# phlash/java-sdr

Hardware: AMD Instinct MI355X
Metric: IQ Msamples/s through FFT+FIR+BPSK demod, 2048-pt frames (higher is better)
Workload: dtype f64

## Files before the change

### include/jsdr_hip.h

```cpp
#ifndef JSDR_HIP_H
#define JSDR_HIP_H

#include <stddef.h>
#include <stdint.h>

#ifdef __cplusplus
extern "C" {
#endif

#define JSDR_OK 0
#define JSDR_ERR (-1)

const char *jsdr_last_error(void);
int jsdr_version(void);
int jsdr_device_count(int *count);
int jsdr_set_device(int device);
int jsdr_get_device(int *device);
int jsdr_device_name(char *buf, int cap);
int jsdr_malloc(void **dev, size_t bytes);
int jsdr_free(void *dev);
int jsdr_live_resources(int64_t *device_buffers, int64_t *device_bytes, int64_t *pinned_buffers, int64_t *streams_and_events);
int jsdr_memset(void *dev, int value, size_t bytes);
int jsdr_memcpy_h2d(void *dev, const void *host, size_t bytes);
int jsdr_memcpy_d2h(void *host, const void *dev, size_t bytes);
// ... 94 lines not shown
int jsdr_bpsk_blob_info(const void *blob_host, size_t bytes, jsdr_bpsk_blob_info_t *out);
int jsdr_bpsk_state_kernel_ms(jsdr_bpsk *h, double *pack_ms, double *unpack_ms);
int jsdr_bpsk_acq_last_launch(jsdr_bpsk *h, int64_t *fwd_frames, int64_t *inv_frames);
int jsdr_bpsk_channel_info(jsdr_bpsk *h, int *ninputs, int *nchannels);
int jsdr_bpsk_set_channel_tuning(jsdr_bpsk *h, int channel, double tuning_hz);
int jsdr_bpsk_set_channel_mode(jsdr_bpsk *h, int channel, int do_fft, int do_up);
int jsdr_bpsk_get_channel_control(jsdr_bpsk *h, int channel, double *tuning_hz, int *do_fft, int *do_up);
int jsdr_bpsk_receive_f32(jsdr_bpsk *h, const float *iq_host);
int jsdr_bpsk_receive_i16(jsdr_bpsk *h, const int16_t *raw_host, int ic, int qc);
int jsdr_bpsk_batch_i16(jsdr_bpsk *h, const int16_t *raw_dev, int64_t stream_stride_i16,
                        int64_t nsamples, int ic, int qc, void *stream);
int jsdr_bpsk_batch_f32(jsdr_bpsk *h, const float *iq_dev, int64_t stream_stride_f32, int64_t nsamples, void *stream);
int jsdr_bpsk_set_cu_share(jsdr_bpsk *h, int wgs_per_cu);
int jsdr_bpsk_pair_shares(jsdr_bpsk *h, int *fft_wgs_per_cu, int *bpsk_wgs_per_cu);
int jsdr_bpsk_last_launch(jsdr_bpsk *h, int64_t *work_items, int64_t *workgroups);
int jsdr_bpsk_sync(jsdr_bpsk *h);
enum { JSDR_BPSK_NCOUNTERS = 10 };
int jsdr_bpsk_get_counters(jsdr_bpsk *h, int stream, int32_t out[JSDR_BPSK_NCOUNTERS]);
int jsdr_bpsk_get_bits(jsdr_bpsk *h, int stream, int8_t *bits_host, int cap, int *nbits);
int jsdr_bpsk_get_fec(jsdr_bpsk *h, int stream, int idx, int32_t *rc, int32_t *bit_index, uint8_t out_host[256]);
int jsdr_bpsk_get_fec_count(jsdr_bpsk *h, int stream, int *count);
int jsdr_bpsk_get_decoded(jsdr_bpsk *h, int stream, uint8_t out_host[256]);
int jsdr_bpsk_get_trace(jsdr_bpsk *h, int stream, double *out_host, int64_t cap_pairs, int64_t *npairs);
int jsdr_bpsk_get_state(jsdr_bpsk *h, int stream, double out[18]);
typedef struct jsdr_bpsk_snapshot {
    int64_t frames;
    int32_t counters[JSDR_BPSK_NCOUNTERS];
    int32_t nbits;
    double state[18];
    uint8_t decoded[256];
// ... 92 lines not shown
```

### java-sdr_amd/binding.py

```python
import ctypes as C
import os
import re

import numpy as np

HERE = os.path.dirname(os.path.abspath(__file__))
ROOT = os.path.dirname(HERE)
_SO = os.environ.get("JSDR_LIB") or os.path.join(HERE, "libjsdr_hip.so")


class JsdrError(RuntimeError):
    pass


def library_path():
    return _SO


def _declared_symbols():
    hdr = open(os.path.join(ROOT, "include", "jsdr_hip.h")).read()
    hdr = re.sub(r"/\*.*?\*/", " ", hdr, flags=re.S)
    return sorted(set(re.findall(r"\b(jsdr_[a-z0-9_]+)\s*\(", hdr)))


# ... 361 lines not shown
def fec_decode_dev(raw_dev, nblocks, out_dev, rc_dev, stream=None):
    _check(lib().jsdr_fec_decode_batch(_addr(raw_dev), C.c_int64(nblocks), _addr(out_dev), _addr(rc_dev),
                                       C.c_void_p(stream)), "jsdr_fec_decode_batch")


COUNTER_NAMES = ["cntRaw", "cntDS", "cntBit", "cntFEC", "cntDec", "dmErrBits", "dmCorr", "dmMaxCorr", "decodeOK",
                 "centreBin"]


class BpskSnapshot(C.Structure):
    _fields_ = [("frames", C.c_int64), ("counters", C.c_int32 * 10), ("nbits", C.c_int32), ("state", C.c_double * 18),
                ("decoded", C.c_uint8 * 256), ("bits", C.c_int8 * 512)]


def bpsk_table(which):
    out = np.empty(65, np.float64)
    _check(lib().jsdr_bpsk_table(which, _addr(out), 65), "jsdr_bpsk_table")
    return out[:27 if which == 0 else 65].copy()


class Bpsk:

    def __init__(self, rate=96000, blen=8192, size=4, tuning=12000, do_fft=0, do_up=0, nstreams=1,
                 max_batch_samples=None, variant="exact"):
        self.samples = blen // size
        self.nstreams = nstreams
        self.max_batch = max_batch_samples or self.samples
        self.h = C.c_void_p()
        _check(lib().jsdr_bpsk_create(C.byref(self.h), rate, self.samples, tuning, do_fft, do_up, nstreams,
                                      C.c_int64(self.max_batch)), "jsdr_bpsk_create")
        if variant != "exact":
            _check(lib().jsdr_bpsk_set_variant(self.h, {"exact": 0, "fast": 1}[variant]), "jsdr_bpsk_set_variant")

# ... 65 lines not shown
               "jsdr_bpsk_recover_uncertified")
        return rec.value

    def set_cu_share(self, wgs_per_cu):
        _check(lib().jsdr_bpsk_set_cu_share(self.h, int(wgs_per_cu)), "jsdr_bpsk_set_cu_share")

    def pair_shares(self):
        a, b = C.c_int(), C.c_int()
        _check(lib().jsdr_bpsk_pair_shares(self.h, C.byref(a), C.byref(b)), "jsdr_bpsk_pair_shares")
        return a.value, b.value

    def last_launch(self):
        a, b = C.c_int64(), C.c_int64()
        _check(lib().jsdr_bpsk_last_launch(self.h, C.byref(a), C.byref(b)), "jsdr_bpsk_last_launch")
        return a.value, b.value

    def sync(self):
        _check(lib().jsdr_bpsk_sync(self.h), "jsdr_bpsk_sync")

    def set_tuning(self, tuning_hz):
        _check(lib().jsdr_bpsk_set_tuning(self.h, C.c_double(tuning_hz)), "jsdr_bpsk_set_tuning")

    def set_mode(self, do_fft, do_up):
        _check(lib().jsdr_bpsk_set_mode(self.h, int(do_fft), int(do_up)), "jsdr_bpsk_set_mode")

    def reconfigure(self, tuning_hz, do_fft, do_up):
        _check(lib().jsdr_bpsk_reconfigure(self.h, C.c_double(tuning_hz), int(do_fft), int(do_up)), "jsdr_bpsk_reconfigure")

    def control(self):
        t, f, u = C.c_double(), C.c_int(), C.c_int()
# ... 497 lines not shown
```

### java-sdr_amd/csrc/bpsk_fm.hip

```cpp
#include "bpsk_units.h"
#include <math.h>
#include <stddef.h>
#include <stdlib.h>

namespace jsdr {
namespace fm { __constant__ BpskConst c_bpsk; }
using fm::c_bpsk;
}
#include "bpsk_matched.h"

namespace jsdr {


template <bool FAST>
__global__ __launch_bounds__(512) void k_matched(MatchedArgs a)
{
    extern __shared__ __align__(16) unsigned char smem[];
    double2 *X = reinterpret_cast<double2 *>(smem);
    const int s = blockIdx.y;
    const long long G = a.tile0 + 4160LL * blockIdx.x;
    const double2 *dm = a.dm + (long long)s * a.dm_stride;
    {
        constexpr int NLD = (64 + 4160 + 511) / 512;
        double2 v[NLD];
// ... 115 lines not shown
    const int s = u >> 5, i = u & 31;
    if (s >= hi.nstreams || i >= 26) return;
    const long long n = hi.nsamples - 26 + i;
    int2 v;
    if (n < 0) {
        v = hi.hist_old[(long long)s * 32 + (26 + n)];
    } else {
        const int w = hi.raw[(long long)s * hi.stride_pairs + n];
        const int si = java_short_add((int)(short)(w & 0xffff), hi.ic);
        const int sq = java_short_add(w >> 16, hi.qc);
        v = make_int2((si & 0xffff) | (sq << 16), 0);
    }
    hi.hist_new[(long long)s * 32 + i] = v;
}

template <int D, int R, bool MIX, bool DC, bool FAST, bool SMALL = false>
#ifndef JSDR_FM_MINWAVES
#define JSDR_FM_MINWAVES 2
#endif
__global__ __launch_bounds__(FM_THREADS, JSDR_FM_MINWAVES) void k_fm(FmArgs a)
{
    constexpr int RD = D * R, NS = RD - D + 27, NSQ = (NS + 3) / 4;
    constexpr int JOBS = (FM_NT + R - 1) / R, ROUNDS = (JOBS + FM_THREADS - 1) / FM_THREADS;
    extern __shared__ __align__(16) unsigned char smem[];
    double2 *X = reinterpret_cast<double2 *>(smem);
    double *sc = reinterpret_cast<double *>(smem + FM_NT * sizeof(double2));
    for (int i = threadIdx.x; i < 512; i += FM_THREADS) sc[i] = a.sincos[i];
#ifdef JSDR_X_CLK
    unsigned long long clk_acc_[6] = {0, 0, 0, 0, 0, 0}, clk_last_ = 0;
#endif
    const long long nwork = (long long)a.ntiles * a.nstreams;
#pragma unroll 1
    for (long long work = blockIdx.x; work < nwork; work += gridDim.x) {
    const int s = (int)(work / a.ntiles);
    const long long G = a.tile0 + (long long)(65 * FM_NB) * (work % a.ntiles);
    const int jrel0 = (int)(G - 64 - a.g_first);
#ifdef JSDR_X_FM_SMALLSET
    const int *raw = a.raw + (long long)(s & 15) * a.stride_pairs;
// ... 4 lines not shown
    const double2 *dmh_old = a.dmh_old + (long long)s * 64;
    const int Lm1 = a.nsamples - 1, nds = a.nds, P = a.tper;
    const double HOWARD = 0.9 * 32768.0 * (double)I16_2P15_UNSCALE;
    int e0 = 0;
    if constexpr (MIX) {
        const long long v = (long long)a.first_out + (long long)D * jrel0;
        e0 = (int)(((v % P) + P) % P);
    }
    typedef const __attribute__((address_space(4))) double *const_tab_t;
    const_tab_t tb = (const_tab_t)(a.tcs + e0);
    float amx = 0.0f;
    __syncthreads();
#ifdef JSDR_X_CLK
    clk_last_ = __builtin_amdgcn_s_memtime();
#endif
#ifdef JSDR_X_NOFRONT
    if (a.nds < 0)
#endif
#pragma unroll 1
    for (int round = 0; round < ROUNDS; round++) {
        const int job = threadIdx.x + FM_THREADS * round;
        const int t0 = R * job;
        if (t0 >= FM_NT) break;
        const int j0 = jrel0 + t0;
        const int n0 = a.first_out + D * j0 - 26;
        const bool none = j0 + R <= 0 || j0 >= nds || nds <= 0;
        const bool regular = j0 >= 0 && j0 + R <= nds;
        if (!none) {
            int4 W[NSQ];
            const int *wp = raw + n0;
// ... 30 lines not shown
                if (q == 0) {
#pragma unroll
                    for (int r = 0; r < R; r++) {
                        const int kv = (kv4[r / 4] >> (8 * (r % 4))) & 0xff;
                        vc[r] = sc[kv];
                        vs[r] = sc[256 + kv];
                    }
                }
#pragma unroll
                for (int t = 3; t >= 0; t--) {
                    const int m = 4 * q + t;
                    if (m < NS) {
                        const int w = (t == 0) ? w4.x : (t == 1) ? w4.y : (t == 2) ? w4.z : w4.w;
                        double di, dq;
                        fm_convert_2p15(w, a.ic, a.qc, DC, di, dq, FAST ? &amx : nullptr);
                        if constexpr (MIX) {
                            di = di * tb[2 * m];
                            dq = dq * tb[2 * m + 1];
                        }
#pragma unroll
                        for (int r = 0; r < R; r++) {
                            if (m >= D * r && m <= D * r + 26) {
                                const int age = D * r + 26 - m;
                                const double tp = ds_tap(age);
                                const bool same = age == 0 || ((kDsPow2Mask >> age) & 1);
                                if (FAST || same) {
                                    ai[r] = __builtin_fma(di, tp, ai[r]);
                                    aq[r] = __builtin_fma(dq, tp, aq[r]);
                                } else {
                                    ai[r] += di * tp;
                                    aq[r] += dq * tp;
                                }
                            }
                        }
                    }
                }
#ifndef JSDR_FM_NOPIN
#pragma unroll
                for (int r = 0; r < R; r++) asm volatile("" : "+v"(ai[r]), "+v"(aq[r])::"memory");
                if constexpr (FAST) asm volatile("" : "+v"(amx));
                __builtin_amdgcn_sched_barrier(0);
#endif
            }
            if (regular) {
#pragma unroll
// ... 17 lines not shown
                        val.y = r == 0 ? oq[0] : r == 1 ? oq[1] : r == 2 ? oq[2] : r == 3 ? oq[3] : oq[R - 1];
                    } else if (j >= -64 && j < 0) {
                        val = dmh_old[64 + j];
                    }
                    if (t < FM_NT) X[t] = val;
                }
            }
        } else {
#pragma unroll 1
            for (int r = 0; r < R; r++) {
                const int t = t0 + r, j = j0 + r;
                const double2 val = (j >= -64 && j < 0) ? dmh_old[64 + j] : make_double2(0.0, 0.0);
                if (t < FM_NT) X[t] = val;
            }
        }
    }
    if constexpr (FAST) {
#pragma unroll
        for (int off = 32; off >= 1; off >>= 1) amx = fmaxf(amx, __shfl_xor(amx, off, 64));
        if ((threadIdx.x & 63) == 0 && amx > 0.0f) atomicMax(a.amax + s, __float_as_int(amx));
    }
    FM_CLK(1);
    __syncthreads();
    FM_CLK(3);
    if (jrel0 + FM_NT > nds - 64) {
        double2 *dmh_new = a.dmh_new + (long long)s * 64;
        for (int t = 64 + threadIdx.x; t < FM_NT; t += FM_THREADS) {
            const int j = jrel0 + t;
            if (j >= nds - 64 && j < nds && j >= 0) dmh_new[j - (nds - 64)] = X[t];
        }
// ... 121 lines not shown

int launch_dm_history(double2 *dm, long long dm_stride, long long nds, int nstreams, hipStream_t st)
{
    hipLaunchKernelGGL(k_dm_history, dim3((unsigned)nstreams), dim3(64), 0, st, dm, dm_stride, nds, nstreams);
    return launched();
}

int launch_fm_prep(const EdgeArgs &ea, const HistArgs &ha, const ScatterArgs &sc, hipStream_t st)
{
    hipLaunchKernelGGL(k_fm_prep, dim3((unsigned)(((long long)ea.nstreams * (4 * FM_EDGE + 32) + sc.bytes[0] + sc.bytes[1] + 255) / 256)),
                       dim3(256), 0, st, ea, ha, sc);
    return launched();
}

template <int D, int R>
static int launch_fm_t(const FmArgs &a_in, bool mix, bool dc, bool fast, int nstreams, hipStream_t st, long long *items, long long *grid_out)
{
    const size_t lds = (size_t)FM_NT * sizeof(double2) + 512 * sizeof(double);
    const long long span = 65LL * FM_NB;
    const long long ntiles = (a_in.g_first + a_in.nds - a_in.tile0 + span - 1) / span;
    FmArgs a = a_in;
    a.ntiles = (int)ntiles;
    a.nstreams = nstreams;
    static const long long grid_cap = [] {
        const char *e = knob("JSDR_FM_GRID");
        return e ? atoll(e) : 0LL;
    }();
    long long gx = ntiles * nstreams;
    if (grid_cap > 0 && gx > grid_cap) gx = grid_cap;
    if (a.grid_limit > 0 && gx > a.grid_limit) gx = a.grid_limit;
    *items = ntiles * nstreams;
    *grid_out = gx;
    const dim3 grid((unsigned)gx), block(FM_THREADS);
#define JSDR_FM_LAUNCH(MIX, DC, FAST, SMALL)                                                                    \
    do {                                                                                                        \
        JSDR_LDS_ATTR((k_fm<D, R, MIX, DC, FAST, SMALL>), lds);                                                 \
        hipLaunchKernelGGL((k_fm<D, R, MIX, DC, FAST, SMALL>), grid, block, lds, st, a);                        \
    } while (0)
    if (!fast && a.nds <= FM_THREADS && ntiles == 1) {
        if (mix) { if (dc) JSDR_FM_LAUNCH(true, true, false, true); else JSDR_FM_LAUNCH(true, false, false, true); }
        else { if (dc) JSDR_FM_LAUNCH(false, true, false, true); else JSDR_FM_LAUNCH(false, false, false, true); }
    } else if (fast) {
        if (mix) { if (dc) JSDR_FM_LAUNCH(true, true, true, false); else JSDR_FM_LAUNCH(true, false, true, false); }
        else { if (dc) JSDR_FM_LAUNCH(false, true, true, false); else JSDR_FM_LAUNCH(false, false, true, false); }
    } else {
        if (mix) { if (dc) JSDR_FM_LAUNCH(true, true, false, false); else JSDR_FM_LAUNCH(true, false, false, false); }
        else { if (dc) JSDR_FM_LAUNCH(false, true, false, false); else JSDR_FM_LAUNCH(false, false, false, false); }
    }
#undef JSDR_FM_LAUNCH
    return launched();
}

int launch_fm(const FmArgs &a, int decim, bool mix, bool dc, bool fast, int nstreams, hipStream_t st, long long *items, long long *grid)
{
    switch (decim) {
        case 4: return launch_fm_t<4, 5>(a, mix, dc, fast, nstreams, st, items, grid);
        case 5: return launch_fm_t<5, 4>(a, mix, dc, fast, nstreams, st, items, grid);
        case 10: return launch_fm_t<10, 4>(a, mix, dc, fast, nstreams, st, items, grid);
        case 20: return launch_fm_t<20, 4>(a, mix, dc, fast, nstreams, st, items, grid);
    }
    set_error("bpsk: unsupported decimation %d", decim);
    return JSDR_ERR;
}

void bpsk_fm_clocks_report()
{
#ifdef JSDR_X_CLK
    {
        static unsigned long long cc[256][64];
        if (hipMemcpyFromSymbol(cc, HIP_SYMBOL(g_fm_clk), sizeof(cc)) == hipSuccess) {
            static const char *nm[6] = {"-", "front half", "-", "barrier front", "matched", "barrier matched"};
            for (int i = 0; i < 6; i++) {
                if (i == 0 || i == 2) continue;
                fprintf(stderr, "k_fm clk %-16s", nm[i]);
// ... 19 lines not shown
```

### java-sdr_amd/csrc/bpsk_handle.hip

```cpp
#include "bpsk_kernels.h"
#include "bpsk_fec.h"
#include "bpsk_fft.h"
#include "bpsk_chan.h"
#include "bpsk_pst.h"
#include "bpsk_sched.h"
#include "bpsk_blob.h"
#include "bpsk_state.h"
#include <math.h>
#include <cmath>
#include <atomic>
#include <memory>
#include <thread>
#include <stddef.h>
#include <stdlib.h>
#include <vector>

static const float h_ds_half[14] = {-6.103515625000e-004F, -1.220703125000e-004F, +2.380371093750e-003F,
                                    +6.164550781250e-003F, +7.324218750000e-003F, +7.629394531250e-004F,
                                    -1.464843750000e-002F, -3.112792968750e-002F, -3.225708007813e-002F,
                                    -1.617431640625e-003F, +6.463623046875e-002F, +1.502380371094e-001F,
                                    +2.231445312500e-001F, +2.518310546875e-001F};
static const float h_dm_half[33] = {
    -0.0101130691F, -0.0086975143F, -0.0038246093F, +0.0033563764F, +0.0107237026F, +0.0157790936F, +0.0164594107F,
    +0.0119213911F, +0.0030315224F, -0.0076488191F, -0.0164594107F, -0.0197184277F, -0.0150109226F, -0.0023082460F,
// ... 49 lines not shown
    bool hist_is_float = false;
    DevBuf<int> hist_bad;
    DevBuf<int> amax;
    DevBuf<SnapPack> snap_dev;
    DevBuf<int> fm_edges;
    DevBuf<float2> fm_edges_f32;
    bool f32_batch = false;
    DevBuf<double2> dm, y[2];
    int y_cur = 0;
    DevBuf<double2> dmh[2], tcs;
    int dmh_cur = 0;
    int tab_cur = 0;
    bool halo_in_dmh = false;
    bool use_fm = true;
    long long last_fm_items = 0, last_fm_grid = 0;
    int share_wgs_per_cu = 0;
    int num_cu = 0;
    int variant = 0;
    double fast_ey = 0.0;
    double margin_scale = 1.0;
    double argmax_scale = 1.0;
    const char *front_name = "k_front";
    const char *tail_name = "k_tail";
    const char *fec_name = "k_fec_bpsk";
    bool ktu_uploaded = false;
    std::thread worker;
    bool prefetch_on = true;
    long long sched_sync = 0, sched_prefetched = 0;
    Stream tail_stream;
    Event ev_matched;
// ... 962 lines not shown
    JSDR_REQUIRE(L > 0 && L <= h->max_batch, "bpsk: nsamples=%lld outside (0, max_batch_samples=%lld]", L, h->max_batch);
    JSDR_REQUIRE((stride_i16 & 1) == 0 && (h->nstreams == 1 || stride_i16 >= 2 * L),
                 "bpsk: stream stride %lld too small for %lld samples", stride_i16, L);
    JSDR_REQUIRE(!h->do_fft || (L % h->nsf) == 0, "bpsk: FFT-acquire mode needs whole frames (%lld %% %d != 0)", L, h->nsf);
    JSDR_REQUIRE(h->variant == 0 || raw_dev, "bpsk: the fast variant takes int16 input (its certification pass re-reads the raw samples)");
    JSDR_REQUIRE(h->seam != SEAM_TO_TUNE || L >= 26, "bpsk: the first tune-mode call after FFT-acquire frames needs at least 26 samples "
                 "(the input history is rebuilt from them)");
    if (rawf_dev && h->f32_batch && h->use_fm && !h->fm_edges_f32.p && (h->decim == 4 || h->decim == 5 || h->decim == 10 || h->decim == 20))
        if (h->fm_edges_f32.alloc((size_t)h->nstreams * 4 * FM_EDGE) != JSDR_OK) return JSDR_ERR;
    if (!h->do_fft && h->seam != SEAM_TO_TUNE && hist_form(h, rawf_dev != nullptr, h->nstreams, st) != JSDR_OK) return JSDR_ERR;
    const int first_out = h->decim - 1 - h->dsCnt;
    const long long g_first = h->n_ds;
    unsigned char kh0[26], mh0[26];
    memcpy(kh0, h->h_khist, 26);
    memcpy(mh0, h->h_mhist, 26);
    const long long nds = build_schedule(h, L);
    JSDR_REQUIRE(nds <= h->max_ds, "bpsk: internal: %lld decimated samples exceed capacity %lld", nds, h->max_ds);
    const int f0 = h->cur.f0;
    const long long n0 = h->cur.n0;
    if (h->n_in == 0) memset(h->h_mhist, f0, 26);
    bool split = false;
    if (!h->do_fft) {
        split = h->cur.mix < 0 || h->seam == SEAM_TO_TUNE;
        for (int i = 0; i < 26 && !split; i++) split = h->h_mhist[i] != (unsigned char)f0;
    }
    const bool std_decim = h->decim == 4 || h->decim == 5 || h->decim == 10 || h->decim == 20;
    const int fm_rd = h->decim == 4 ? 20 : h->decim * 4;
    const bool per_ok = !h->do_fft && !split && h->cur.mix == 1 && h->cur.tper > 0 && fm_rd % h->cur.tper == 0;
    const bool fm_ok = h->use_fm && std_decim && !h->do_fft && !split && nds > 0 && L <= 0x3fffffffLL &&
                       ((raw_dev && !rawf_dev) || (rawf_dev && h->f32_batch && h->variant == 0 && h->fm_edges_f32.p)) && (h->cur.mix == 0 || per_ok);
// ... 167 lines not shown
        ma.edges = h->fm_edges.p;
        ma.tcs = tcs_p;
        ma.tper = h->cur.mix ? h->cur.tper : 1;
        ma.kvco = kvco_p;
        ma.sincos = h->sincos.p;
        ma.dmh_old = h->dmh[h->dmh_cur].p;
        ma.dmh_new = h->dmh[h->dmh_cur ^ 1].p;
        ma.y = h->y[h->y_cur].p + Y_PAD;
        ma.y_stride = h->y_stride;
        ma.nds = (int)nds;
        ma.g_first = g_first;
        ma.tile0 = first_block(g_first);
        ma.first_out = first_out;
        ma.amax = h->amax.p;
        ma.grid_limit = h->share_wgs_per_cu * h->num_cu;
        if (rawf_dev) {
            EdgeF32Args ea;
            ea.rawf = fa.rawf;
            ea.stride_pairs = fa.stride_pairs;
            ea.nsamples = (int)L;
            ea.hist = fa.hist;
            ea.edges = h->fm_edges_f32.p;
            ea.nstreams = S;
            const HistArgs ha = hist_args(h, nullptr, fa.rawf, fa.stride_pairs, L, 0, 0, S);
            ProfScope psh(h, PK_PREP, st);
            if (launch_fm_prep_f32(ea, ha, st) != JSDR_OK) return JSDR_ERR;
            hist_done = true;
        } else {
            EdgeArgs ea;
            ea.raw = fa.raw;
// ... 8 lines not shown
            const HistArgs ha = hist_args(h, fa.raw, nullptr, fa.stride_pairs, L, ic, qc, S);
            ProfScope psh(h, PK_PREP, st);
            if (launch_fm_prep(ea, ha, sc, st) != JSDR_OK) return JSDR_ERR;
            hist_done = true;
        }
        ProfScope ps(h, PK_FM, st);
        if (rawf_dev) {
            FmF32Args mf;
            mf.a = ma;
            mf.rawf = fa.rawf;
            mf.edges = h->fm_edges_f32.p;
            h->front_name = "k_fm_f32";
            if (launch_fm_f32(mf, h->decim, h->cur.mix != 0, S, st, &h->last_fm_items, &h->last_fm_grid) != JSDR_OK) return JSDR_ERR;
        } else {
        h->front_name = "k_fm";
        if (launch_fm(ma, h->decim, h->cur.mix != 0, (ic != 0) || (qc != 0), h->variant != 0, S, st, &h->last_fm_items, &h->last_fm_grid) != JSDR_OK)
            return JSDR_ERR;
        }
        h->dmh_cur ^= 1;
    } else if (nds > 0) {
        ProfScope ps(h, PK_FRONT, st);
        const bool fast = false;
        const char *front = launch_front(fa, h->decim, S, fast, st);
        if (!front) return JSDR_ERR;
        h->front_name = front;
    }
    if (!h->do_fft && hist_done) h->hist_cur ^= 1;
    if (!h->do_fft && !hist_done)
        if (run_hist_in(h, hist_args(h, fa.raw, fa.rawf, fa.stride_pairs, L, ic, qc, S), st) != JSDR_OK) return JSDR_ERR;
    const int yb = h->y_cur;
    if (wait_tail(h, yb, st) != JSDR_OK) return JSDR_ERR;
// ... 119 lines not shown
                for (int i = 0; i < 4096; i++)
                    if (w[2 * i + 1] && w[2 * i] - t0 > (e1 - t0) / 10) late++;
                fprintf(stderr, "[jsdr] k_acq_fwd %d workgroups: %d started late (> 10 %% into the launch); first end %.3f ms, last end %.3f ms after the first start\n",
                        n, late, (double)(e0 - t0) / 1e5, (double)(e1 - t0) / 1e5);
            }
        }
        long long tot = 0;
        for (int k = 0; k < 8; k++) tot += c[k];
        for (int k = 0; k < 8; k++)
            fprintf(stderr, "[jsdr] k_front_fft phase %-20s %12lld ticks  %5.1f %%\n", names[k], c[k],
                    tot ? 100.0 * (double)c[k] / (double)tot : 0.0);
    }
}

extern "C" {

int jsdr_bpsk_create(jsdr_bpsk **out, int rate, int nsamples_per_frame, int tuning_hz, int do_fft, int do_up,
                     int nstreams, int64_t max_batch_samples)
{
    JSDR_REQUIRE(out, "jsdr_bpsk_create: null handle pointer");
    *out = nullptr;
    JSDR_REQUIRE(rate >= 1, "jsdr_bpsk_create: rate %d", rate);
    const int decim = rate / 9600 > 0 ? rate / 9600 : 1;
    JSDR_REQUIRE(nsamples_per_frame > 0 && nstreams > 0 && nstreams <= 65535, "jsdr_bpsk_create: bad geometry");
    if (max_batch_samples < nsamples_per_frame) max_batch_samples = nsamples_per_frame;
    FftFront front = FRONT_NONE;
    if (do_fft) {
        int force_gen = -1;
        if (const char *e = knob("JSDR_ACQG")) force_gen = atoi(e) != 0;
        front = fft_front_kind(nsamples_per_frame, decim, false, force_gen);
// ... 49 lines not shown
              h->ds_taps_dev.alloc(32) == JSDR_OK &&
              h->dmh[0].alloc(S * 64) == JSDR_OK && h->dmh[1].alloc(S * 64) == JSDR_OK && h->hist_bad.alloc(1) == JSDR_OK && h->amax.alloc(S) == JSDR_OK && h->fm_edges.alloc(S * 4 * FM_EDGE) == JSDR_OK && h->snap_dev.alloc(1) == JSDR_OK && h->tcs.alloc(2 * (256 + FM_TABLE_SLACK)) == JSDR_OK;
    if (ok && nstreams == 1) {
        const size_t need = sizeof(float) * 2 * (size_t)nsamples_per_frame + ((size_t)h->max_batch + 26) + (size_t)h->max_ds +
                            (do_fft ? sizeof(double2) * (size_t)h->max_ds : 0) + sizeof(double2) * (256 + FM_TABLE_SLACK) + 8 * 64;
        const size_t arena = (need + 63) & ~(size_t)63;
        if (arena <= ((size_t)8 << 20) && h->pin.alloc(arena + sizeof(SnapPack))) h->pin_bytes = arena;
        else (void)hipGetLastError();
    }
    if (!ok) {
        jsdr_bpsk_destroy(h);
        return JSDR_ERR;
    }
    std::vector<double> sc(512);
    for (int n = 0; n < 256; n++) {
        double arg = n * 2.0 * TUNER_PI / 256;
        sc[n] = (double)cosl((long double)arg);
        sc[256 + n] = (double)sinl((long double)arg);
    }
    BpskConst bc;
    memset(&bc, 0, sizeof(bc));
    double sync[SYNC_N];
    (void)jsdr_bpsk_table(0, bc.ds_taps, 32);
    (void)jsdr_bpsk_table(1, bc.dm_taps, 96);
    (void)jsdr_bpsk_table(2, sync, SYNC_N);
    for (int i = 0; i < SYNC_N; i++) bc.sync[i] = sync[i] > 0.0 ? 1 : -1;
    if (do_fft) {
        if (fft_mode_alloc(h, front, false) != JSDR_OK) {
            set_error("jsdr_bpsk_create: FFT-mode initialisation failed");
            jsdr_bpsk_destroy(h);
            return JSDR_ERR;
        }
        if (const char *e = knob("JSDR_ACQ3")) h->acq_mode = atoi(e) != 0 ? 1 : 0;
// ... 151 lines not shown

int jsdr_bpsk_pair_shares(jsdr_bpsk *h, int *fft_wgs_per_cu, int *bpsk_wgs_per_cu)
{
    JSDR_REQUIRE(h && fft_wgs_per_cu && bpsk_wgs_per_cu, "jsdr_bpsk_pair_shares: null argument");
    const bool pays = !h->do_fft && h->rate == 96000 && h->nsf == 2048 && h->variant == 0 && h->nstreams >= 8192;
    *fft_wgs_per_cu = pays ? 2 : 0;
    *bpsk_wgs_per_cu = pays ? 1 : 0;
    return JSDR_OK;
}

int jsdr_bpsk_last_launch(jsdr_bpsk *h, int64_t *work_items, int64_t *workgroups)
{
    JSDR_REQUIRE(h && work_items && workgroups, "jsdr_bpsk_last_launch: null argument");
    *work_items = h->last_fm_items;
    *workgroups = h->last_fm_grid;
    return JSDR_OK;
}

int jsdr_bpsk_receive_i16(jsdr_bpsk *h, const int16_t *raw_host, int ic, int qc)
{
    JSDR_REQUIRE(h && raw_host, "jsdr_bpsk_receive_i16: null argument");
    JSDR_REQUIRE(!h->pst, "jsdr_bpsk_receive_i16: a tuned handle (jsdr_bpsk_create_tuned) takes batches only; receive() is the 1-stream "
                 "form of jsdr_bpsk_create");
    JSDR_REQUIRE(h->nstreams == 1 || (h->nch > 0 && h->nin == 1),
                 "jsdr_bpsk_receive_i16: handle has %d streams; receive() is the 1-stream form (or a 1-input channel handle)",
                 h->nstreams);
    h->pin_call = true;
    h->pin_off = 0;
    int rc = JSDR_OK;
    const size_t fb = sizeof(int16_t) * 2 * (size_t)h->nsf;
// ... 317 lines not shown
    }
    set_error("jsdr_bpsk_snapshot_read: could not get a stable copy");
    return JSDR_ERR;
}

int jsdr_bpsk_profile_enable(jsdr_bpsk *h, int on)
{
    JSDR_REQUIRE(h, "jsdr_bpsk_profile_enable: null handle");
    h->prof_on = on != 0;
    return JSDR_OK;
}

int jsdr_bpsk_table(int which, double *out, int cap)
{
    JSDR_REQUIRE(out, "jsdr_bpsk_table: null argument");
    const int n = which == 0 ? 27 : ((which == 1 || which == 2) ? 65 : 0);
    JSDR_REQUIRE(n > 0 && cap >= n, "jsdr_bpsk_table: table %d needs room for %d values", which, n);
    if (which == 0) {
        for (int i = 0; i < 14; i++) out[i] = out[26 - i] = (double)h_ds_half[i];
    } else if (which == 1) {
        for (int i = 0; i < 33; i++) out[i] = out[64 - i] = (double)h_dm_half[i];
    } else {
        int sr = 0x7f;
        for (int i = 0; i < 65; i++) {
            out[i] = (sr & 64) ? 1.0 : -1.0;
            int v = sr & 0x48;
            v ^= v >> 4;
            v ^= v >> 2;
            v ^= v >> 1;
            sr = ((sr << 1) | (v & 1)) & 0xffff;
        }
    }
    return JSDR_OK;
// ... 835 lines not shown
```

### java-sdr_amd/csrc/bpsk_kernels.h

```cpp
#pragma once
#include "common.h"
#include "bpsk_fft.h"

namespace jsdr {

enum { DS_N = 27, DM_N = 65, HIST_BITS = 5200, MIN_TRIG = 8, SYNC_N = 65 };
enum { Y_PAD = 1024 };
#ifndef JSDR_FM_NB
#define JSDR_FM_NB 62
#endif
enum { FM_NB = JSDR_FM_NB, FM_NT = 64 + 65 * FM_NB, FM_THREADS = 512, FM_TABLE_SLACK = 128, FM_EDGE = 128 };

struct BpskConst {
    double ds_taps[32];
    double dm_taps[96];
    signed char sync[72];
};
int bpsk_upload_constants(const BpskConst &bc);

struct TailState {
    double dmEnergy[8];
    double dmEnergyOut;
    double lastI, lastQ;
    double energy1, energy2;
// ... 66 lines not shown
    const double2 *tcs;
    int tper;
    const unsigned char *kvco;
    const double *sincos;
    const double2 *dmh_old;
    double2 *dmh_new;
    double2 *y;
    long long y_stride;
    int nds;
    long long g_first;
    long long tile0;
    int first_out;
    int *amax;
    int ntiles, nstreams;
    int grid_limit;
};

struct EdgeArgs {
    const int *raw;
    long long stride_pairs;
    int nsamples, ic, qc, dc;
    const int2 *hist;
    int *edges;
    int nstreams;
};
struct ScatterArgs {
    const unsigned char *src[2];
    unsigned char *dst[2];
    int bytes[2];
};
// ... 52 lines not shown

bool front_reg_enabled();
const char *launch_front(const FrontArgs &fa, int decim, int nstreams, bool fast, hipStream_t st);
int launch_front_split(const FrontArgs &fa, const unsigned short *ktu9, const double *sc9, int decim, const FftFrontState *dhist,
                       int nstreams, hipStream_t st);
int launch_seam_hist(const int2 *hist, int is_float, const double *sincos, const SeamHist &sh, FftFrontState *st, FftFrontState *st2,
                     int nstreams, hipStream_t stream);
int launch_seam_q(double2 *dm, long long dm_stride, const double2 *dm2, long long dm2_stride, int J, int nstreams, hipStream_t st);
int launch_chan_seam_hist(const int2 *hist, int is_float, const double *sc9, const ChanSeamHist &sh, FftFrontState *st, double *qcol,
                          int ninputs, hipStream_t stream);
int launch_hist_in(const HistArgs &ha, hipStream_t st);
int launch_hist_convert(int2 *hist, int nstreams, int to_float, int *bad, hipStream_t st);
int launch_matched(const MatchedArgs &ma, int nstreams, hipStream_t st);
int launch_dm_history(double2 *dm, long long dm_stride, long long nds, int nstreams, hipStream_t st);
int launch_fm_prep(const EdgeArgs &ea, const HistArgs &ha, const ScatterArgs &sc, hipStream_t st);
int launch_fm(const FmArgs &a, int decim, bool mix, bool dc, bool fast, int nstreams, hipStream_t st, long long *items, long long *grid);
int launch_fm_prep_f32(const EdgeF32Args &ea, const HistArgs &ha, hipStream_t st);
int launch_fm_f32(const FmF32Args &a, int decim, bool mix, int nstreams, hipStream_t st, long long *items, long long *grid);
const char *launch_tail(const TailArgs &ta, bool cert, hipStream_t st);
bool sync_t_applies(int max_bits);
int launch_sync_t(const SyncArgs &sa, const SyncFinArgs &sf, int nstreams, hipStream_t st);
int launch_sync(const SyncArgs &sa, long long nds, int nstreams, hipStream_t st);
int launch_sync_fin(const SyncArgs &sa, const SyncFinArgs &sf, int nstreams, hipStream_t st);
int launch_reset_maxcorr(TailState *st, int nstreams, hipStream_t stream);
int launch_reset_maxcorr_chan(TailState *st, int nin, int nch, int ch, hipStream_t stream);
int launch_pack_slots(unsigned char *slots, long long slot_bytes, int slot_bits, int trig_cap, const TailState *st, const int *nbits,
                      const signed char *bitlog, long long bitlog_stride, const int *trig_count, const int *trig_bits, const int *fec_rc,
                      const unsigned char *fec_data, const int *fec_last, const int *cnt_dec, int n_in, int n_ds, int nstreams, hipStream_t stream);
void bpsk_debug_clocks_report();

}
// ... 14 lines not shown
```

### java-sdr_amd/csrc/bpsk_sched.h

```cpp
#pragma once
#include "bpsk_tuner.h"
#include <vector>

namespace jsdr {
#pragma GCC visibility push(hidden)

enum { SCHED_HIST = 26 };

long long vco_walk(double &vco, int &ds, int decim, long long L, std::vector<unsigned char> &kvco);

struct VcoSchedule {
    bool valid = false;
    double vco0 = 0.0;
    int ds0 = 0, decim = 0;
    long long L = -1;
    double vco1 = 0.0;
    int ds1 = 0;
    std::vector<unsigned char> kvco;
};
bool vco_schedule(VcoSchedule &v, double vco, int ds, int decim, long long L);

struct ScheduleKey {
    double tu0 = 0.0, inc = 0.0, vco0 = 0.0;
    int ds0 = 0, decim = 0;
// ... 1 lines not shown
    bool do_fft = false, first = false;
    unsigned char khist0[SCHED_HIST] = {0};
    bool same_call(const ScheduleKey &o) const;
    bool operator==(const ScheduleKey &o) const { return same_call(o) && first == o.first; }
};

struct Schedule {
    bool valid = false;
    ScheduleKey key;
    double tu1 = 0.0, vco1 = 0.0;
    int ds1 = 0;
    int mix = 1;
    int f0 = 1;
    long long n0 = 0;
    int tper = 0;
    long long nds = 0;
    std::vector<unsigned char> ktu;
    std::vector<unsigned char> kvco;
    std::vector<double2> tcs;
};
enum { SCHED_TABLE_SLACK = 128 };

inline void schedule_key(Schedule &sc, const ScheduleKey &key)
{
    sc.valid = false;
    sc.key = key;
}
inline bool schedule_matches(const Schedule &sc, const ScheduleKey &key) { return sc.valid && sc.key == key; }
void compute_schedule(Schedule &sc, const double *sincos);

// ... 40 lines not shown
```

### java-sdr_amd/csrc/bpsk_sched.hip

```cpp
#include "bpsk_sched.h"
#include <thread>

namespace jsdr {

struct TunerWalk {
    double tu, inc;
    unsigned char *kt;
    long long nmix = 0;
};
template <bool TUNER>
static long long walk(TunerWalk *t, double &vco_io, int &ds_io, int decim, long long L, std::vector<unsigned char> &kvco)
{
    kvco.clear();
    kvco.reserve((size_t)(L / decim + 2));
    double tu = TUNER ? t->tu : 0.0, vco = vco_io;
    const double inc = TUNER ? t->inc : 0.0;
    int cnt = ds_io;
    long long nmix = 0;
    for (long long n = 0; n < L; n++) {
        if (TUNER) {
            tuner_advance(tu, inc);
            int k = 0;
            if (tu > 0.0) {
                k = tuner_k9(tu);
// ... 54 lines not shown
        memset(t.kt, 0, (size_t)L);
        sc.nds = walk<false>(nullptr, sc.vco1, sc.ds1, key.decim, L, sc.kvco);
    } else {
        sc.nds = walk<true>(&t, sc.vco1, sc.ds1, key.decim, L, sc.kvco);
    }
    sc.mix = (t.nmix == L) ? 1 : (t.nmix == 0 ? 0 : -1);
    sc.f0 = sc.mix == 0 ? 0 : 1;
    sc.n0 = L;
    if (sc.mix < 0) {
        double tu = key.tu0;
        sc.f0 = tuner_step(tu, key.inc) != 256;
        sc.n0 = sc.f0 ? t.nmix : L - t.nmix;
    }
    sc.tu1 = t.tu;
    sc.tper = 0;
    if (!key.do_fft && sc.mix == 1) {
        const long long off = key.first ? SCHED_HIST : 0;
        const unsigned char *k = sc.ktu.data() + off;
        const long long len = L + SCHED_HIST - off;
        const long long head = len < 1024 ? len : 1024;
        for (int p = 1; p <= 256 && p < len; p++) {
            if (!period_holds(k, head, p)) continue;
            if (period_holds(k, len, p)) {
                sc.tper = p;
                sc.tcs.resize((size_t)p + SCHED_TABLE_SLACK);
                for (int e = 0; e < p + SCHED_TABLE_SLACK; e++) {
                    const int i = (int)(((e - off) % p + p) % p);
                    const int kk = k[i];
                    sc.tcs[(size_t)e] = make_double2(sincos[kk], sincos[256 + kk]);
                }
            }
            break;
        }
    }
    sc.valid = true;
}

bool ChanKey::operator==(const ChanKey &o) const
{
    return tu0 == o.tu0 && inc == o.inc && L == o.L && first == o.first && memcmp(hist0, o.hist0, sizeof(hist0)) == 0;
}

void chan_compute(ChanSchedule &c)
{
    const long long L = c.key.L;
// ... 72 lines not shown
```

### java-sdr_amd/csrc/bpsk_tuner.h

```cpp
#pragma once
#include "common.h"

namespace jsdr {

constexpr double TUNER_PI = 3.14159265358979323846;

inline double tuner_inc(double tuning, int rate) { return 2.0 * TUNER_PI * tuning / (double)rate; }

__host__ __device__ inline void tuner_advance(double &tu, double inc)
{
    const double two_pi = 2.0 * TUNER_PI;
    tu += inc;
    if (tu > two_pi) tu -= two_pi;
}

__host__ __device__ inline int tuner_k9(double tu)
{
    const double two_pi = 2.0 * TUNER_PI;
    return tu > 0.0 ? (int)(tu * (double)256 / two_pi) % 256 : 256;
}

__host__ __device__ inline int tuner_step(double &tu, double inc)
{
    tuner_advance(tu, inc);
    return tuner_k9(tu);
}

__host__ __device__ inline int vco_step(double &vco)
{
    const double two_pi = 2.0 * TUNER_PI;
    const double vinc = 2.0 * TUNER_PI * 1200.0 / (double)9600;
    vco += vinc;
    if (vco > two_pi) vco -= two_pi;
    return (int)(vco * (double)256 / two_pi) % 256;
}

}
```

Before: 243,500.

## Specialise k_fm front-end for period-8 tuner with exact 0/±1 mixing factors

When the tuner schedule has period 8 and its factors match the quarter-rate pattern (cos/sin equal to 0 or ±1 at known phases), the host detects the rotation and launches a phase-specialised k_fm variant. That variant skips the mixing multiply for unit factors and drops the FMAs against zero factors at compile time, cutting f64 arithmetic in the decimating front end. A static_assert checks the tap exactness the FMA substitution relies on. The cost is more template instantiations and a runtime branch between two phase forms per tile. It only applies for decimation 10 with a period-8 tuner.

```diff
diff --git a/include/jsdr_hip.h b/include/jsdr_hip.h
--- a/include/jsdr_hip.h
+++ b/include/jsdr_hip.h
@@ -132,6 +132,7 @@
 int jsdr_bpsk_set_cu_share(jsdr_bpsk *h, int wgs_per_cu);
 int jsdr_bpsk_pair_shares(jsdr_bpsk *h, int *fft_wgs_per_cu, int *bpsk_wgs_per_cu);
 int jsdr_bpsk_last_launch(jsdr_bpsk *h, int64_t *work_items, int64_t *workgroups);
+int jsdr_bpsk_fm_form(jsdr_bpsk *h, int *specialised, int *phase);
 int jsdr_bpsk_sync(jsdr_bpsk *h);
 enum { JSDR_BPSK_NCOUNTERS = 10 };
 int jsdr_bpsk_get_counters(jsdr_bpsk *h, int stream, int32_t out[JSDR_BPSK_NCOUNTERS]);
diff --git a/java-sdr_amd/binding.py b/java-sdr_amd/binding.py
--- a/java-sdr_amd/binding.py
+++ b/java-sdr_amd/binding.py
@@ -399,9 +399,9 @@
 
 
 def bpsk_table(which):
-    out = np.empty(65, np.float64)
-    _check(lib().jsdr_bpsk_table(which, _addr(out), 65), "jsdr_bpsk_table")
-    return out[:27 if which == 0 else 65].copy()
+    out = np.empty(256, np.float64)
+    _check(lib().jsdr_bpsk_table(which, _addr(out), 256), "jsdr_bpsk_table")
+    return out[:{0: 27, 1: 65, 2: 65}.get(which, 256)].copy()
 
 
 class Bpsk:
@@ -497,6 +497,11 @@
         a, b = C.c_int64(), C.c_int64()
         _check(lib().jsdr_bpsk_last_launch(self.h, C.byref(a), C.byref(b)), "jsdr_bpsk_last_launch")
         return a.value, b.value
+
+    def fm_form(self):
+        a, b = C.c_int(), C.c_int()
+        _check(lib().jsdr_bpsk_fm_form(self.h, C.byref(a), C.byref(b)), "jsdr_bpsk_fm_form")
+        return bool(a.value), b.value
 
     def sync(self):
         _check(lib().jsdr_bpsk_sync(self.h), "jsdr_bpsk_sync")
diff --git a/java-sdr_amd/csrc/bpsk_fm.hip b/java-sdr_amd/csrc/bpsk_fm.hip
--- a/java-sdr_amd/csrc/bpsk_fm.hip
+++ b/java-sdr_amd/csrc/bpsk_fm.hip
@@ -1,5 +1,7 @@
 #include "bpsk_units.h"
+#include "bpsk_tuner.h"
 #include <math.h>
+#include <type_traits>
 #include <stddef.h>
 #include <stdlib.h>
 
@@ -153,7 +155,17 @@
     hi.hist_new[(long long)s * 32 + i] = v;
 }
 
-template <int D, int R, bool MIX, bool DC, bool FAST, bool SMALL = false>
+constexpr bool ds_taps_are_short()
+{
+    for (int n = 0; n < 14; n++) {
+        const float k = kDsHalf[n] * 32768.0f;
+        if (k != (float)(int)k || k >= 16384.0f || k <= -16384.0f) return false;
+    }
+    return true;
+}
+static_assert(ds_taps_are_short(), "dsFilter: every tap times 2^15 is an integer of magnitude below 2^14 (k_fm's +-1.0 fmas are exact)");
+
+template <int D, int R, bool MIX, bool DC, bool FAST, bool SMALL = false, int PH = -1>
 #ifndef JSDR_FM_MINWAVES
 #define JSDR_FM_MINWAVES 2
 #endif
@@ -161,6 +173,8 @@
 {
     constexpr int RD = D * R, NS = RD - D + 27, NSQ = (NS + 3) / 4;
     constexpr int JOBS = (FM_NT + R - 1) / R, ROUNDS = (JOBS + FM_THREADS - 1) / FM_THREADS;
+    static_assert(PH < 0 || (MIX && !FAST && PH < 4 && (D * R) % 8 == 0 && (65 * FM_NB * D) % 8 == 4),
+                  "k_fm<PH>: the lane span is whole periods and a tile is half a period past the one before");
     extern __shared__ __align__(16) unsigned char smem[];
     double2 *X = reinterpret_cast<double2 *>(smem);
     double *sc = reinterpret_cast<double *>(smem + FM_NT * sizeof(double2));
@@ -195,6 +209,8 @@
 #ifdef JSDR_X_CLK
     clk_last_ = __builtin_amdgcn_s_memtime();
 #endif
+    auto front = [&](auto phc) __attribute__((always_inline)) {
+    constexpr int PHC = decltype(phc)::value;
 #ifdef JSDR_X_NOFRONT
     if (a.nds < 0)
 #endif
@@ -255,9 +271,10 @@
                         const int w = (t == 0) ? w4.x : (t == 1) ? w4.y : (t == 2) ? w4.z : w4.w;
                         double di, dq;
                         fm_convert_2p15(w, a.ic, a.qc, DC, di, dq, FAST ? &amx : nullptr);
+                        const int ci = PHC >= 0 ? tuner8_class(PHC + m, 0) : TC_GEN, cq = PHC >= 0 ? tuner8_class(PHC + m, 1) : TC_GEN;
                         if constexpr (MIX) {
-                            di = di * tb[2 * m];
-                            dq = dq * tb[2 * m + 1];
+                            if (ci == TC_GEN) di = di * tb[2 * m];
+                            if (cq == TC_GEN) dq = dq * tb[2 * m + 1];
                         }
 #pragma unroll
                         for (int r = 0; r < R; r++) {
@@ -265,11 +282,14 @@
                                 const int age = D * r + 26 - m;
                                 const double tp = ds_tap(age);
                                 const bool same = age == 0 || ((kDsPow2Mask >> age) & 1);
-                                if (FAST || same) {
-                                    ai[r] = __builtin_fma(di, tp, ai[r]);
-                                    aq[r] = __builtin_fma(dq, tp, aq[r]);
+                                if (FAST || same || ci != TC_GEN) {
+                                    if (ci != TC_ZERO) ai[r] = __builtin_fma(di, ci == TC_MONE ? -tp : tp, ai[r]);
                                 } else {
                                     ai[r] += di * tp;
+                                }
+                                if (FAST || same || cq != TC_GEN) {
+                                    if (cq != TC_ZERO) aq[r] = __builtin_fma(dq, cq == TC_MONE ? -tp : tp, aq[r]);
+                                } else {
                                     aq[r] += dq * tp;
                                 }
                             }
@@ -317,6 +337,13 @@
                 if (t < FM_NT) X[t] = val;
             }
         }
+    }
+    };
+    if constexpr (PH < 0) {
+        front(std::integral_constant<int, -1>{});
+    } else {
+        if (((e0 + a.trot) & 7) == PH) front(std::integral_constant<int, PH>{});
+        else front(std::integral_constant<int, PH + 4>{});
     }
     if constexpr (FAST) {
 #pragma unroll
@@ -468,8 +495,10 @@
 }
 
 template <int D, int R>
-static int launch_fm_t(const FmArgs &a_in, bool mix, bool dc, bool fast, int nstreams, hipStream_t st, long long *items, long long *grid_out)
-{
+static int launch_fm_t(const FmArgs &a_in, bool mix, bool dc, bool fast, int nstreams, hipStream_t st, long long *items, long long *grid_out,
+                       int *phase)
+{
+    *phase = -1;
     const size_t lds = (size_t)FM_NT * sizeof(double2) + 512 * sizeof(double);
     const long long span = 65LL * FM_NB;
     const long long ntiles = (a_in.g_first + a_in.nds - a_in.tile0 + span - 1) / span;
@@ -486,12 +515,28 @@
     *items = ntiles * nstreams;
     *grid_out = gx;
     const dim3 grid((unsigned)gx), block(FM_THREADS);
-#define JSDR_FM_LAUNCH(MIX, DC, FAST, SMALL)                                                                    \
+#define JSDR_FM_LAUNCH_PH(MIX, DC, FAST, SMALL, PH)                                                             \
     do {                                                                                                        \
-        JSDR_LDS_ATTR((k_fm<D, R, MIX, DC, FAST, SMALL>), lds);                                                 \
-        hipLaunchKernelGGL((k_fm<D, R, MIX, DC, FAST, SMALL>), grid, block, lds, st, a);                        \
+        JSDR_LDS_ATTR((k_fm<D, R, MIX, DC, FAST, SMALL, PH>), lds);                                             \
+        hipLaunchKernelGGL((k_fm<D, R, MIX, DC, FAST, SMALL, PH>), grid, block, lds, st, a);                    \
     } while (0)
-    if (!fast && a.nds <= FM_THREADS && ntiles == 1) {
+#define JSDR_FM_LAUNCH(MIX, DC, FAST, SMALL) JSDR_FM_LAUNCH_PH(MIX, DC, FAST, SMALL, -1)
+    const bool small = !fast && a.nds <= FM_THREADS && ntiles == 1;
+    if constexpr (D == 10) {
+        if (mix && !fast && !small && a.trot >= 0 && a.tper == 8) {
+            const long long v = (long long)a.first_out + (long long)D * (a.tile0 - 64 - a.g_first);
+            const int p0 = (int)((((v % 8) + 8) % 8 + a.trot) & 7);
+            *phase = p0;
+            switch (p0 & 3) {
+                case 0: if (dc) JSDR_FM_LAUNCH_PH(true, true, false, false, 0); else JSDR_FM_LAUNCH_PH(true, false, false, false, 0); break;
+                case 1: if (dc) JSDR_FM_LAUNCH_PH(true, true, false, false, 1); else JSDR_FM_LAUNCH_PH(true, false, false, false, 1); break;
+                case 2: if (dc) JSDR_FM_LAUNCH_PH(true, true, false, false, 2); else JSDR_FM_LAUNCH_PH(true, false, false, false, 2); break;
+                default: if (dc) JSDR_FM_LAUNCH_PH(true, true, false, false, 3); else JSDR_FM_LAUNCH_PH(true, false, false, false, 3); break;
+            }
+            return launched();
+        }
+    }
+    if (small && a.nds <= FM_THREADS && ntiles == 1) {
         if (mix) { if (dc) JSDR_FM_LAUNCH(true, true, false, true); else JSDR_FM_LAUNCH(true, false, false, true); }
         else { if (dc) JSDR_FM_LAUNCH(false, true, false, true); else JSDR_FM_LAUNCH(false, false, false, true); }
     } else if (fast) {
@@ -502,16 +547,18 @@
         else { if (dc) JSDR_FM_LAUNCH(false, true, false, false); else JSDR_FM_LAUNCH(false, false, false, false); }
     }
 #undef JSDR_FM_LAUNCH
+#undef JSDR_FM_LAUNCH_PH
     return launched();
 }
 
-int launch_fm(const FmArgs &a, int decim, bool mix, bool dc, bool fast, int nstreams, hipStream_t st, long long *items, long long *grid)
+int launch_fm(const FmArgs &a, int decim, bool mix, bool dc, bool fast, int nstreams, hipStream_t st, long long *items, long long *grid,
+              int *phase)
 {
     switch (decim) {
-        case 4: return launch_fm_t<4, 5>(a, mix, dc, fast, nstreams, st, items, grid);
-        case 5: return launch_fm_t<5, 4>(a, mix, dc, fast, nstreams, st, items, grid);
-        case 10: return launch_fm_t<10, 4>(a, mix, dc, fast, nstreams, st, items, grid);
-        case 20: return launch_fm_t<20, 4>(a, mix, dc, fast, nstreams, st, items, grid);
+        case 4: return launch_fm_t<4, 5>(a, mix, dc, fast, nstreams, st, items, grid, phase);
+        case 5: return launch_fm_t<5, 4>(a, mix, dc, fast, nstreams, st, items, grid, phase);
+        case 10: return launch_fm_t<10, 4>(a, mix, dc, fast, nstreams, st, items, grid, phase);
+        case 20: return launch_fm_t<20, 4>(a, mix, dc, fast, nstreams, st, items, grid, phase);
     }
     set_error("bpsk: unsupported decimation %d", decim);
     return JSDR_ERR;
diff --git a/java-sdr_amd/csrc/bpsk_handle.hip b/java-sdr_amd/csrc/bpsk_handle.hip
--- a/java-sdr_amd/csrc/bpsk_handle.hip
+++ b/java-sdr_amd/csrc/bpsk_handle.hip
@@ -87,6 +87,7 @@
     bool halo_in_dmh = false;
     bool use_fm = true;
     long long last_fm_items = 0, last_fm_grid = 0;
+    int last_fm_phase = -1;
     int share_wgs_per_cu = 0;
     int num_cu = 0;
     int variant = 0;
@@ -1079,6 +1080,7 @@
     unsigned char kh0[26], mh0[26];
     memcpy(kh0, h->h_khist, 26);
     memcpy(mh0, h->h_mhist, 26);
+    h->last_fm_phase = -1;
     const long long nds = build_schedule(h, L);
     JSDR_REQUIRE(nds <= h->max_ds, "bpsk: internal: %lld decimated samples exceed capacity %lld", nds, h->max_ds);
     const int f0 = h->cur.f0;
@@ -1276,6 +1278,7 @@
         ma.first_out = first_out;
         ma.amax = h->amax.p;
         ma.grid_limit = h->share_wgs_per_cu * h->num_cu;
+        ma.trot = h->cur.mix == 1 ? h->cur.trot : -1;
         if (rawf_dev) {
             EdgeF32Args ea;
             ea.rawf = fa.rawf;
@@ -1314,7 +1317,8 @@
             if (launch_fm_f32(mf, h->decim, h->cur.mix != 0, S, st, &h->last_fm_items, &h->last_fm_grid) != JSDR_OK) return JSDR_ERR;
         } else {
         h->front_name = "k_fm";
-        if (launch_fm(ma, h->decim, h->cur.mix != 0, (ic != 0) || (qc != 0), h->variant != 0, S, st, &h->last_fm_items, &h->last_fm_grid) != JSDR_OK)
+        if (launch_fm(ma, h->decim, h->cur.mix != 0, (ic != 0) || (qc != 0), h->variant != 0, S, st, &h->last_fm_items, &h->last_fm_grid,
+                      &h->last_fm_phase) != JSDR_OK)
             return JSDR_ERR;
         }
         h->dmh_cur ^= 1;
@@ -1464,6 +1468,9 @@
 }
 
 extern "C" {
+
+static double table_cos(int n) { return (double)cosl((long double)(n * 2.0 * TUNER_PI / 256)); }
+static double table_sin(int n) { return (double)sinl((long double)(n * 2.0 * TUNER_PI / 256)); }
 
 int jsdr_bpsk_create(jsdr_bpsk **out, int rate, int nsamples_per_frame, int tuning_hz, int do_fft, int do_up,
                      int nstreams, int64_t max_batch_samples)
@@ -1543,9 +1550,8 @@
     }
     std::vector<double> sc(512);
     for (int n = 0; n < 256; n++) {
-        double arg = n * 2.0 * TUNER_PI / 256;
-        sc[n] = (double)cosl((long double)arg);
-        sc[256 + n] = (double)sinl((long double)arg);
+        sc[n] = table_cos(n);
+        sc[256 + n] = table_sin(n);
     }
     BpskConst bc;
     memset(&bc, 0, sizeof(bc));
@@ -1727,6 +1733,14 @@
     JSDR_REQUIRE(h && work_items && workgroups, "jsdr_bpsk_last_launch: null argument");
     *work_items = h->last_fm_items;
     *workgroups = h->last_fm_grid;
+    return JSDR_OK;
+}
+
+int jsdr_bpsk_fm_form(jsdr_bpsk *h, int *specialised, int *phase)
+{
+    JSDR_REQUIRE(h && specialised && phase, "jsdr_bpsk_fm_form: null argument");
+    *specialised = h->last_fm_phase >= 0;
+    *phase = h->last_fm_phase;
     return JSDR_OK;
 }
 
@@ -2074,9 +2088,11 @@
 int jsdr_bpsk_table(int which, double *out, int cap)
 {
     JSDR_REQUIRE(out, "jsdr_bpsk_table: null argument");
-    const int n = which == 0 ? 27 : ((which == 1 || which == 2) ? 65 : 0);
+    const int n = which == 0 ? 27 : ((which == 1 || which == 2) ? 65 : ((which == 3 || which == 4) ? 256 : 0));
     JSDR_REQUIRE(n > 0 && cap >= n, "jsdr_bpsk_table: table %d needs room for %d values", which, n);
-    if (which == 0) {
+    if (which >= 3) {
+        for (int i = 0; i < 256; i++) out[i] = which == 3 ? table_cos(i) : table_sin(i);
+    } else if (which == 0) {
         for (int i = 0; i < 14; i++) out[i] = out[26 - i] = (double)h_ds_half[i];
     } else if (which == 1) {
         for (int i = 0; i < 33; i++) out[i] = out[64 - i] = (double)h_dm_half[i];
diff --git a/java-sdr_amd/csrc/bpsk_kernels.h b/java-sdr_amd/csrc/bpsk_kernels.h
--- a/java-sdr_amd/csrc/bpsk_kernels.h
+++ b/java-sdr_amd/csrc/bpsk_kernels.h
@@ -104,6 +104,7 @@
     int *amax;
     int ntiles, nstreams;
     int grid_limit;
+    int trot;
 };
 
 struct EdgeArgs {
@@ -186,7 +187,8 @@
 int launch_matched(const MatchedArgs &ma, int nstreams, hipStream_t st);
 int launch_dm_history(double2 *dm, long long dm_stride, long long nds, int nstreams, hipStream_t st);
 int launch_fm_prep(const EdgeArgs &ea, const HistArgs &ha, const ScatterArgs &sc, hipStream_t st);
-int launch_fm(const FmArgs &a, int decim, bool mix, bool dc, bool fast, int nstreams, hipStream_t st, long long *items, long long *grid);
+int launch_fm(const FmArgs &a, int decim, bool mix, bool dc, bool fast, int nstreams, hipStream_t st, long long *items, long long *grid,
+              int *phase);
 int launch_fm_prep_f32(const EdgeF32Args &ea, const HistArgs &ha, hipStream_t st);
 int launch_fm_f32(const FmF32Args &a, int decim, bool mix, int nstreams, hipStream_t st, long long *items, long long *grid);
 const char *launch_tail(const TailArgs &ta, bool cert, hipStream_t st);
diff --git a/java-sdr_amd/csrc/bpsk_sched.h b/java-sdr_amd/csrc/bpsk_sched.h
--- a/java-sdr_amd/csrc/bpsk_sched.h
+++ b/java-sdr_amd/csrc/bpsk_sched.h
@@ -39,6 +39,7 @@
     int f0 = 1;
     long long n0 = 0;
     int tper = 0;
+    int trot = -1;
     long long nds = 0;
     std::vector<unsigned char> ktu;
     std::vector<unsigned char> kvco;
diff --git a/java-sdr_amd/csrc/bpsk_sched.hip b/java-sdr_amd/csrc/bpsk_sched.hip
--- a/java-sdr_amd/csrc/bpsk_sched.hip
+++ b/java-sdr_amd/csrc/bpsk_sched.hip
@@ -92,6 +92,7 @@
     }
     sc.tu1 = t.tu;
     sc.tper = 0;
+    sc.trot = -1;
     if (!key.do_fft && sc.mix == 1) {
         const long long off = key.first ? SCHED_HIST : 0;
         const unsigned char *k = sc.ktu.data() + off;
@@ -107,6 +108,7 @@
                     const int kk = k[i];
                     sc.tcs[(size_t)e] = make_double2(sincos[kk], sincos[256 + kk]);
                 }
+                if (p == 8) sc.trot = tuner8_rotation(sc.tcs.data());
             }
             break;
         }
diff --git a/java-sdr_amd/csrc/bpsk_tuner.h b/java-sdr_amd/csrc/bpsk_tuner.h
--- a/java-sdr_amd/csrc/bpsk_tuner.h
+++ b/java-sdr_amd/csrc/bpsk_tuner.h
@@ -1,5 +1,6 @@
 #pragma once
 #include "common.h"
+#include <string.h>
 
 namespace jsdr {
 
@@ -26,6 +27,29 @@
     return tuner_k9(tu);
 }
 
+enum { TC_GEN = 0, TC_ONE = 1, TC_MONE = 2, TC_ZERO = 3 };
+constexpr int tuner8_class(int ph, int rail)
+{
+    return rail == 0 ? ((ph & 7) == 0 ? TC_ONE : (ph & 7) == 4 ? TC_MONE : TC_GEN)
+                     : ((ph & 7) == 0 ? TC_ZERO : (ph & 7) == 2 ? TC_ONE : (ph & 7) == 6 ? TC_MONE : TC_GEN);
+}
+inline int tuner_factor_class(double v)
+{
+    unsigned long long b;
+    memcpy(&b, &v, sizeof(b));
+    return b == 0x3ff0000000000000ULL ? TC_ONE : b == 0xbff0000000000000ULL ? TC_MONE : (b << 1) == 0 ? TC_ZERO : TC_GEN;
+}
+inline int tuner8_rotation(const double2 *tab)
+{
+    for (int r = 0; r < 8; r++) {
+        bool ok = true;
+        for (int e = 0; e < 8 && ok; e++)
+            ok = tuner_factor_class(tab[e].x) == tuner8_class(e + r, 0) && tuner_factor_class(tab[e].y) == tuner8_class(e + r, 1);
+        if (ok) return r;
+    }
+    return -1;
+}
+
 __host__ __device__ inline int vco_step(double &vco)
 {
     const double two_pi = 2.0 * TUNER_PI;
```

After: 247,000 (median of 6 runs). 1.01x the previous value.
